# EmbodiedVision/diffsdfsim

Measured on AMD Instinct MI355X. Metric: sim steps/sec (fwd+bwd), 1024 batched 3D scenes x 8 SDF bodies, higher is better.
Workload: dtype f64

## Files before the change

diffsdfsim_amd/csrc/launchers.h:

```cpp
#pragma once
#include "dss_device.h"

#include "../../include/diffsdfsim_hip.h"

namespace dss {
int launch_find_contacts(const DssWorld &W, int *nc_out, int *body_out, int *face_out, double *abc_out,
                         double *geom_out, hipStream_t stream);
int launch_find_contacts_all(const DssWorld &W, int *nc_out, int *body_out, int *face_out, double *abc_out,
                             double *geom_out, hipStream_t stream);
int launch_find_contacts_box(const DssWorld &W, int *nc_out, int *body_out, int *face_out, double *abc_out,
                             double *geom_out, hipStream_t stream);
int launch_igr_rounds(const DssWorld &W, hipStream_t stream);
int launch_igr_list(const DssIgrNet &N, const double *pts, const int *lat_idx, const double *latents, int lat_stride,
                    const int *n_dev, int n_cap, int mode, double *sdf, double *grad, hipStream_t stream, int est);
int launch_igr_pair(const DssIgrNet &N, const double *pts_v, const int *lat_v, const int *n_v, double *sdf_v, const double *pts_g,
                    const int *lat_g, const int *n_g, double *sdf_g, double *grad_g, const double *latents, int lat_stride, int n_cap,
                    hipStream_t stream, int est_v, int est_g);
void launch_bwd_pre_all(const DssWorld &W, const DssAdjoint &A, hipStream_t stream);
int lcp_contact_backward_rows(const double *Mblk, const double *A, const double *cop, const int *cbody, const int *nc,
                              const int *active, int B, int nb, int neq, int maxc, int fric_dirs, const double *x,
                              const double *lam, const double *slack, const double *nu, const double *dl_dx, double *dMblk,
                              double *dpvec, double *dcop, double *dA, double *db, int rows, const int *slot, void *stream);
bool lcp_dense_group_fits(int nz, int nineq, int neq);
int launch_lcp_dense_group_forward(const double *Q, const double *p, const double *G, const double *h, const double *A, const double *b,
                                   const double *F, int B, int nz, int nineq, int neq, double eps, int not_improved_lim, int max_iter,
                                   int check_spd, double *zhat, double *lam, double *slack, double *nu, int *iters, int *status,
                                   hipStream_t stream);
int launch_lcp_dense_group_backward(const double *Q, const double *G, const double *A, const double *F, int B, int nz, int nineq, int neq,
                                    const double *zhat, const double *lam, const double *slack, const double *nu, const double *dl_dz,
                                    double *dQ, double *dp, double *dG, double *dh, double *dA, double *db, double *dF, hipStream_t stream);
}
```

diffsdfsim_amd/csrc/narrowphase.hip:

```cpp
#ifndef DSS_ALL_SHAPES
#define DSS_ALL_SHAPES 0
#endif
#ifndef DSS_BOX_ONLY
#define DSS_BOX_ONLY 0
#endif
#if !DSS_ALL_SHAPES && !DSS_BOX_ONLY
#define DSS_STAMPS np
#endif

#include "launchers.h"
#include "np_common.h"

namespace {
constexpr int NP_WAVES = 3;
constexpr int OV_RUN = 256;
constexpr int OV_NT = 256;
__global__ void __launch_bounds__(OV_NT) overlap_kernel(DssWorld W)
{
    __shared__ unsigned char s_ok[64 * 63 / 2];
    __shared__ unsigned char s_big[64];
    const int nb = W.nb, nup = nb * (nb - 1) / 2, np = npairs_of(nb);
    const int sc = blockIdx.x, tid = threadIdx.x, lane = tid & 63, wv = tid >> 6;
    if (!W.active[sc]) return;
    const bool few = (long)W.B * np <= 256L * NP_WAVES;
    if (tid < nb) {
        const int nf = W.mesh_nf[W.mesh_id[(size_t)sc * nb + tid]];
        s_big[tid] = nf > WAVE_ITEM_MAX_FACES || (few && nf > 2048);
    }
#if DSS_ALL_SHAPES
    __shared__ unsigned char s_igr[64];
    if (tid < nb) s_igr[tid] = W.shape_type[(size_t)sc * nb + tid] == DSS_SHAPE_IGR;
#endif
    for (int up = wv; up < nup; up += OV_NT / 64) {
        int i, j;
        upair_of(up, nb, i, j);
        int ok = !W.no_contact[i * nb + j];
        if (ok) {
            BodyD A, Bd;
            load_body(W, sc, i, A);
            load_body(W, sc, j, Bd);
            for (int dir = 0; dir < 2 && ok; ++dir) {
                const BodyD &src = dir ? Bd : A, &dst = dir ? A : Bd;
                const double s = dst.g.shape.scale;
                Region reg;
                region_of(src.g, dst.g, 1e-9, reg);
                const double *vbox = W.vch_box + (size_t)W.mesh_vch_off[src.mesh] * 6;
                const int nch = (src.nv + OV_RUN - 1) / OV_RUN;
                int found = 0;
                for (int cb0 = 0; cb0 < nch && !found; cb0 += 64) {
                    const int ch = cb0 + lane;
                    unsigned long long m = __ballot(ch < nch && box_hits(reg, vbox + (size_t)ch * 6));
                    while (m && !found) {
                        const int b = __ffsll((long long)m) - 1;
                        m &= m - 1;
                        int hit = 0;
#pragma unroll
                        for (int sub = 0; sub < OV_RUN / 64; ++sub) {
                            const int v = (cb0 + b) * OV_RUN + sub * 64 + lane;
                            if (v < src.nv) {
                                double p[3];
                                to_frame(src.g, dst.g, W.verts + (size_t)(src.voff + v) * 3, p);
                                hit |= (-s <= p[0] && p[0] <= s && -s <= p[1] && p[1] <= s && -s <= p[2] && p[2] <= s);
                            }
                        }
                        found = __ballot(hit) != 0ull;
                    }
                }
                ok = found;
            }
        }
        if (lane == 0) {
            s_ok[up] = (unsigned char)ok;
            W.ovl[((size_t)sc * nb + i) * nb + j] = ok;
            if (!ok) {
                W.pc_count[(size_t)sc * np + i * (nb - 1) + (j - 1)] = 0;
                W.pc_count[(size_t)sc * np + j * (nb - 1) + i] = 0;
            }
        }
    }
    __syncthreads();
    if (tid == 0) {
        int cnt[2] = {0, 0};
#if DSS_ALL_SHAPES
        int nig = 0;
        for (int up = 0, i = 0, j = 1; up < nup; ++up, upair_next(nb, i, j)) {
            if (s_ok[up] && (s_igr[i] || s_igr[j])) nig += 2;
        }
        if (nig) {
            int at = atomicAdd(W.n_pairs + 6, nig);
            for (int up = 0, i = 0, j = 1; up < nup; ++up, upair_next(nb, i, j)) {
                if (s_ok[up] && (s_igr[i] || s_igr[j])) {
                    s_ok[up] = 0;
                    if (W.igr_list && at + 2 <= W.igr_items_cap) {
                        W.igr_list[at++] = sc * np + i * (nb - 1) + (j - 1);
                        W.igr_list[at++] = sc * np + j * (nb - 1) + i;
                    } else atomicOr(W.overflow + sc, 32);
                }
            }
        }
#endif
        for (int up = 0, i = 0, j = 1; up < nup; ++up, upair_next(nb, i, j)) {
            if (s_ok[up]) { ++cnt[s_big[i] ? 0 : 1]; ++cnt[s_big[j] ? 0 : 1]; }
        }
        const int cap = W.B * np;
        const unsigned long long old = atomicAdd(reinterpret_cast<unsigned long long *>(W.n_pairs),
                                                 (unsigned long long)(unsigned)cnt[0] | ((unsigned long long)(unsigned)cnt[1] << 32));
        int at[2] = {(int)(old & 0xffffffffull), (int)(old >> 32)};
        for (int up = 0, i = 0, j = 1; up < nup; ++up, upair_next(nb, i, j)) {
            if (s_ok[up]) {
                const int li = s_big[i] ? 0 : 1, lj = s_big[j] ? 0 : 1;
                W.pair_list[(size_t)li * cap + at[li]++] = sc * np + i * (nb - 1) + (j - 1);
                W.pair_list[(size_t)lj * cap + at[lj]++] = sc * np + j * (nb - 1) + i;
            }
        }
    }
}

template <class G> __device__ int narrow_pair(const DssWorld &W, ScratchT<G> &S, int item, int slot_id)
{
    STAMP(0);
    item = dss_uniform(item); slot_id = dss_uniform(slot_id);
    const int np = npairs_of(W.nb);
    const int sc = item / np, dp = item % np, tid = G::tid();
    int a, b;
    pair_of(dp, W.nb, a, b);
    int *pc_count = W.pc_count + (size_t)sc * np + dp;
    BodyD A, Bd;
    load_body(W, sc, a, A);
    load_body(W, sc, b, Bd);
    const int MC = W.max_cand;
    int *__restrict__ cface = W.cand_face + (size_t)slot_id * 2 * MC, *__restrict__ kface = cface + MC;
    int *__restrict__ cstate = W.cand_state + (size_t)slot_id * MC;
    double *__restrict__ cb = W.cand_buf + (size_t)slot_id * DSS_CAND_FIELDS * MC;
    const double *__restrict__ m_verts = W.verts, *__restrict__ m_fcent = W.fcent;
    const int *__restrict__ m_faces = W.faces;
    const double sB = Bd.g.shape.scale;

    double R12[9], t12[3];
    pair_transform(A.g, Bd.g, R12, t12);

    int ncand = 0, over = 0;
    Region reg;
    region_of(A.g, Bd.g, 1e-9, reg);
    const double *fbox = W.fch_box + (size_t)W.mesh_fch_off[A.mesh] * 6;
    constexpr int RUN = 256;
    const int nch = (A.nf + RUN - 1) / RUN, lane = tid & 63, wv = tid >> 6;
    auto cull_face = [&](const double *c) -> int { return centroid_in_cube(R12, t12, c, sB); };
// ... 332 lines not shown
    DSS_KERNARG_REF(DssWorld, W, W_arg);
    __shared__ NpScratch S;
    __shared__ int s_item;
    const int cap = W.B * npairs_of(W.nb), seg = DEFERRED ? 2 : 0;
    {
        const int n = W.n_pairs[DEFERRED ? 4 : 0];
        const int *list = W.pair_list + (size_t)seg * cap;
        for (;;) {
            __syncthreads();
            if (threadIdx.x == 0) s_item = atomicAdd(W.n_pairs + (DEFERRED ? 5 : 2), 1);
            __syncthreads();
            const int it = s_item;
            if (it >= n) break;
            narrow_pair<BlockGroup>(W, S.blk, list[it], (int)blockIdx.x * BlockGroup::NW);
        }
    }
    if (DEFERRED) return;
    __syncthreads();
    const int n = W.n_pairs[1], lane = threadIdx.x & 63;
    const int *list = W.pair_list + cap;
    ScratchT<WaveGroup> &Sw = S.wav[threadIdx.x >> 6];
    for (;;) {
        int it = 0;
        if (lane == 0) it = atomicAdd(W.n_pairs + 3, 1);
        it = __shfl(it, 0);
        if (it >= n) break;
        const int item = list[it];
        if (narrow_pair<WaveGroup>(W, Sw, item, (int)(blockIdx.x * BlockGroup::NW + (threadIdx.x >> 6))) && lane == 0)
            W.pair_list[(size_t)2 * cap + atomicAdd(W.n_pairs + 4, 1)] = item;
        dss_wave_sync();
    }
}

__global__ void __launch_bounds__(64) compact_contacts_kernel(DssWorld W, int *nc_out, int *body_out, int *face_out,
                                                               double *abc_out, double *geom_out)
{
    constexpr int MAXSLOT = 64 * 63;
    __shared__ int s_off[MAXSLOT + 1];
    __shared__ short s_a[MAXSLOT], s_b[MAXSLOT];
    __shared__ unsigned char s_neg[MAXSLOT];
    const int sc = blockIdx.x, lane = threadIdx.x, nb = W.nb, np = npairs_of(nb), MP = W.max_pc, MX = W.maxc;
    if (!W.active[sc]) return;
    int run = 0;
    for (int base = 0; base < np; base += 64) {
        const int slot = base + lane;
        int cnt = 0, a = 0, b = 0;
        if (slot < np) {
            int i, j;
            upair_of(slot >> 1, nb, i, j);
            a = (slot & 1) ? j : i; b = (slot & 1) ? i : j;
            cnt = W.pc_count[(size_t)sc * np + a * (nb - 1) + (b < a ? b : b - 1)];
        }
        const int fwd = __shfl_up(cnt, 1, 64);
        if ((slot & 1) && fwd < 0) cnt = 0;
        if (slot < np) s_neg[slot] = cnt < 0;
        if (cnt < 0) cnt = -cnt;
        int incl = cnt;
        for (int d = 1; d < 64; d <<= 1) { const int o = __shfl_up(incl, d, 64); if (lane >= d) incl += o; }
        if (slot < np) { s_off[slot] = run + incl - cnt; s_a[slot] = (short)a; s_b[slot] = (short)b; }
        run += __shfl(incl, 63, 64);
    }
    if (lane == 0) s_off[np] = run;
    __syncthreads();
    const int total = run < MX ? run : MX;
    for (int o = lane; o < total; o += 64) {
        int lo = 0, hi = np;
        while (hi - lo > 1) { const int mid = (lo + hi) >> 1; if (s_off[mid] <= o) lo = mid; else hi = mid; }
        const int a = s_a[lo], b = s_b[lo], k = o - s_off[lo];
        const size_t dp = (size_t)sc * np + a * (nb - 1) + (b < a ? b : b - 1);
        const int *pf = W.pc_face + dp * MP;
        const double *pabc = W.pc_abc + dp * 3 * MP, *pg = W.pc_geom + dp * 10 * MP;
        const int face = s_neg[lo] ? -1 - pf[k] : pf[k];
        double abc[3], geo[10];
        for (int f = 0; f < 3; ++f) abc[f] = pabc[(size_t)f * MP + k];
        for (int f = 0; f < 10; ++f) geo[f] = pg[(size_t)f * MP + k];
        body_out[(size_t)sc * 2 * MX + o] = a;
        body_out[(size_t)sc * 2 * MX + MX + o] = b;
        face_out[(size_t)sc * MX + o] = face;
        for (int f = 0; f < 3; ++f) abc_out[((size_t)sc * 3 + f) * MX + o] = abc[f];
        for (int f = 0; f < 10; ++f) geom_out[((size_t)sc * 10 + f) * MX + o] = geo[f];
    }
    if (lane == 0) {
        if (run > MX) atomicOr(W.overflow + sc, 8);
        nc_out[sc] = total;
    }
}

}

namespace dss {
static inline int np_grid(int B, int nb)
{
    const long items = (long)B * nb * (nb - 1);
    return (int)(items < 256 * NP_WAVES ? items : 256 * NP_WAVES);
}
#if DSS_ALL_SHAPES
int launch_find_contacts_all(const DssWorld &W, int *nc_out, int *body_out, int *face_out, double *abc_out,
                             double *geom_out, hipStream_t stream)
{
#elif DSS_BOX_ONLY
int launch_find_contacts_box(const DssWorld &W, int *nc_out, int *body_out, int *face_out, double *abc_out,
                             double *geom_out, hipStream_t stream)
{
#else
int launch_find_contacts(const DssWorld &W, int *nc_out, int *body_out, int *face_out, double *abc_out,
                         double *geom_out, hipStream_t stream)
{
    if (W.shape_rare) return launch_find_contacts_all(W, nc_out, body_out, face_out, abc_out, geom_out, stream);
    if (W.shape_box) return launch_find_contacts_box(W, nc_out, body_out, face_out, abc_out, geom_out, stream);
#endif
    static_assert(BlockGroup::HCAP <= BlockGroup::BT * MAX_CPT && WaveGroup::HCAP <= WaveGroup::BT * MAX_CPT, "mover registers");
    if (W.max_cand < 1 || W.nb < 1) return DSS_E_UNSUPPORTED;
    if (W.nb < 2) {
        hipLaunchKernelGGL(compact_contacts_kernel, dim3(W.B), dim3(64), 0, stream, W, nc_out, body_out, face_out, abc_out, geom_out);
        return hipGetLastError() == hipSuccess ? DSS_OK : DSS_E_UNSUPPORTED;
    }
    const int nup = W.nb * (W.nb - 1) / 2, np = W.nb * (W.nb - 1);
    (void)hipMemsetAsync(W.n_pairs, 0, 8 * sizeof(int), stream);
    hipLaunchKernelGGL(overlap_kernel, dim3(W.B), dim3(OV_NT), 0, stream, W);
    const int grid = np_grid(W.B, W.nb);
    hipLaunchKernelGGL(narrowphase_kernel<false>, dim3(grid), dim3(NT), 0, stream, W);
    hipLaunchKernelGGL(narrowphase_kernel<true>, dim3(grid < 64 ? grid : 64), dim3(NT), 0, stream, W);
#if DSS_ALL_SHAPES
    if (W.igr_list) { const int rc = launch_igr_rounds(W, stream); if (rc) return rc; }
#endif
    hipLaunchKernelGGL(compact_contacts_kernel, dim3(W.B), dim3(64), 0, stream, W, nc_out, body_out, face_out, abc_out, geom_out);
    return hipGetLastError() == hipSuccess ? DSS_OK : DSS_E_UNSUPPORTED;
}
}

#if !DSS_ALL_SHAPES && !DSS_BOX_ONLY
extern "C" int dss_np_slots(int B, int nb) { return dss::np_grid(B, nb) * 4; }
#endif
```

diffsdfsim_amd/csrc/np_common.h:

```cpp
#pragma once
#include <math.h>
#include <stdlib.h>

#include "../../include/diffsdfsim_hip.h"
#include "contact_geom.h"
#include "diag_stamps.h"
#include "wave_utils.h"

namespace {
using namespace dss;

constexpr int NT = 256;
constexpr int MAX_CPT = 8;
constexpr int HULL3_MAX = 48;
constexpr int WAVE_ITEM_MAX_FACES = 1 << 30;
#define STAMP(i) DSS_STAMP(G::tid() == 0, (size_t)item * 8 + (i))

__device__ inline int npairs_of(int nb) { return nb * (nb - 1); }
__device__ inline void pair_of(int dp, int nb, int &a, int &b)
{
    a = dp / (nb - 1);
    const int r = dp % (nb - 1);
    b = r < a ? r : r + 1;
}
// ... 728 lines not shown
    return 0;
}
template <class G>
__device__ __noinline__ void emit_unfiltered(const DssWorld &W, int sc, int dp, int ncon, int over, const int *kface, const double *cb, int MC)
{
    const int np = npairs_of(W.nb), tid = G::tid(), MP = W.max_pc;
    int *pf = W.pc_face + ((size_t)sc * np + dp) * MP;
    double *pabc = W.pc_abc + ((size_t)sc * np + dp) * 3 * MP, *pg = W.pc_geom + ((size_t)sc * np + dp) * 10 * MP;
    int nout = ncon;
    if (nout > MP) { over |= 4; nout = MP; }
    for (int k = tid; k < nout; k += G::BT) {
        pf[k] = kface[k];
        for (int i = 0; i < 3; ++i) {
            pabc[(size_t)i * MP + k] = CB(F_CABC + i, k);
            pg[(size_t)i * MP + k] = CB(F_NORMAL + i, k);
            pg[(size_t)(3 + i) * MP + k] = CB(F_P1 + i, k);
            pg[(size_t)(6 + i) * MP + k] = CB(F_P2 + i, k);
        }
        pg[(size_t)9 * MP + k] = CB(F_PEN, k);
    }
    if (tid == 0) { W.pc_count[(size_t)sc * np + dp] = -nout; if (over) atomicOr(W.overflow + sc, over); }
}

template <class G>
__device__ __forceinline__ int filter_and_emit(const DssWorld &W, ScratchT<G> &S, int item, int sc, int dp, int ncon, int over,
                                               int *__restrict__ cface, int *__restrict__ kface, int *__restrict__ cstate,
                                               double *__restrict__ cb, int MC)
{
    const int np = npairs_of(W.nb), tid = G::tid();
    int *pc_count = W.pc_count + (size_t)sc * np + dp;
#include "np_filter_emit.inc"
}

}
```

diffsdfsim_amd/csrc/step.hip:

```cpp
#include <math.h>

#include "../../include/diffsdfsim_hip.h"
#include "contact_geom.h"
#include "launchers.h"
#include "wave_utils.h"

namespace {
using namespace dss;

__global__ void __launch_bounds__(64) begin_kernel(DssWorld W)
{
    const int sc = blockIdx.x * 64 + threadIdx.x;
    if (sc >= W.B) return;
    if (W.step_mask && !W.step_mask[sc]) { W.active[sc] = 0; return; }
    const double t = W.t[sc];
    W.t_end[sc] = t + W.dt;
    W.dt_try[sc] = (t + W.dt) - t;
    W.active[sc] = 1;
    if (W.had_contacts) W.had_contacts[sc] = 0;
    atomicAdd(W.n_active, 1);
}

__global__ void __launch_bounds__(64) assemble_kernel(DssWorld W)
{
    const int sc = blockIdx.x, lane = threadIdx.x, nb = W.nb, MX = W.maxc;
    if (!W.active[sc]) return;
    const int ND = W.fric_dirs / 2, NF = 3 * (1 + ND) + 8;
    double dt = W.dt_try[sc];
    if (W.toc_diff && W.toc[sc]) { const double l = W.last_dt[sc]; dt = -l + (l + dt); }
    if (lane == 0) { W.dt_use[sc] = dt; W.invalid[sc] = 0; }
    if (lane < nb) {
        const size_t bi = (size_t)sc * nb + lane;
        double ps[7], v[6];
        for (int i = 0; i < 7; ++i) { ps[i] = W.pose[bi * 7 + i]; W.pose0[bi * 7 + i] = ps[i]; }
        for (int i = 0; i < 6; ++i) { v[i] = W.vel[bi * 6 + i]; W.vel0[bi * 6 + i] = v[i]; }
        double Iw[9];
        world_inertia(ps, W.inertia + bi * 9, Iw);
// ... 19 lines not shown
        for (int i = 0; i < 3; ++i) { n[i] = g[(size_t)i * MX + c]; p1[i] = g[(size_t)(3 + i) * MX + c]; p2[i] = g[(size_t)(6 + i) * MX + c]; }
        friction_dirs(n, ND, D);
        for (int i = 0; i < 3; ++i) {
            cop[(size_t)i * MX + c] = n[i];
            for (int k = 0; k < ND; ++k) cop[(size_t)(3 * (k + 1) + i) * MX + c] = D[k][i];
        }
        const int o = 3 * (1 + ND);
        for (int i = 0; i < 3; ++i) { cop[(size_t)(o + i) * MX + c] = p1[i]; cop[(size_t)(o + 3 + i) * MX + c] = p2[i]; }
        const size_t i1 = (size_t)sc * nb + b1, i2 = (size_t)sc * nb + b2;
        cop[(size_t)(o + 6) * MX + c] = 0.5 * (W.fric[i1] + W.fric[i2]);
        const double *v1 = W.vel + i1 * 6, *v2 = W.vel + i2 * 6;
        double c1[3], c2[3], jv = 0.0;
        cross(p1, n, c1);
        cross(p2, n, c2);
        for (int i = 0; i < 3; ++i) jv += c1[i] * v1[i] + n[i] * v1[3 + i] - c2[i] * v2[i] - n[i] * v2[3 + i];
        cop[(size_t)(o + 7) * MX + c] = jv * (0.5 * (W.restitution[i1] + W.restitution[i2]));
    }
}

__global__ void __launch_bounds__(64) integrate_kernel(DssWorld W)
{
    const int sc = blockIdx.x, lane = threadIdx.x, nb = W.nb;
    if (!W.active[sc]) return;
    if (lane < nb) {
        const size_t bi = (size_t)sc * nb + lane;
        double v[6], out[7];
        for (int i = 0; i < 6; ++i) { v[i] = -W.x[(size_t)sc * 6 * nb + 6 * lane + i]; W.vel[bi * 6 + i] = v[i]; }
        const double dt = W.dt_use[sc];
        integrate_pose(W.pose0 + bi * 7, v, dt, out);
        for (int i = 0; i < 7; ++i) W.pose[bi * 7 + i] = out[i];
    }
}

struct NewContacts {
    int *nc, *body, *face;
    double *abc, *geom;
};

__global__ void __launch_bounds__(64) decide_kernel(DssWorld W, NewContacts N)
{
    const int sc = blockIdx.x, lane = threadIdx.x, nb = W.nb, MX = W.maxc;
    if (!W.active[sc]) return;
    if (lane == 0 && W.overflow[sc]) atomicOr(W.n_active, DSS_N_ACTIVE_OVERFLOW);
    const double dt_try = W.dt_try[sc];
    const bool tiny = !W.strict_no_pen && dt_try < W.dt / 1024.0;
    const bool accept = !W.invalid[sc] || tiny;
    if (accept) {
        const int nc_new = N.nc[sc], nc_old = W.nc[sc];
        __shared__ unsigned s_pairs[64 * 64 / 32];
        for (int w = lane; w < (nb * nb + 31) / 32; w += 64) s_pairs[w] = 0u;
        __syncthreads();
        for (int c = lane; c < nc_old; c += 64) {
            const int bit = W.c_body[(size_t)sc * 2 * MX + c] * nb + W.c_body[(size_t)sc * 2 * MX + MX + c];
            atomicOr(&s_pairs[bit >> 5], 1u << (bit & 31));
        }
        __syncthreads();
        int toc = 0;
        for (int c = lane; c < nc_new; c += 64) {
            const int a = N.body[(size_t)sc * 2 * MX + c], b = N.body[(size_t)sc * 2 * MX + MX + c];
            const int ab = a * nb + b, ba = b * nb + a;
            toc |= !(((s_pairs[ab >> 5] >> (ab & 31)) | (s_pairs[ba >> 5] >> (ba & 31))) & 1u);
        }
        toc = __ballot(toc) != 0ull;
        const bool escaped = W.invalid[sc] != 0;
        if (escaped) toc = W.toc[sc];
        const int slot = W.nsub[sc];
        if (W.tp_pose && slot >= W.max_sub && lane == 0) { atomicOr(W.overflow + sc, 16); atomicOr(W.n_active, DSS_N_ACTIVE_OVERFLOW); }
        if (W.tp_pose && slot < W.max_sub) {
            const size_t rec = (size_t)slot * W.B + sc;
            if (lane < nb) {
                for (int i = 0; i < 7; ++i) W.tp_pose[(rec * nb + lane) * 7 + i] = W.pose0[((size_t)sc * nb + lane) * 7 + i];
                for (int i = 0; i < 6; ++i) {
                    W.tp_vel[(rec * nb + lane) * 6 + i] = W.vel0[((size_t)sc * nb + lane) * 6 + i];
                    W.tp_x[rec * 6 * nb + 6 * lane + i] = W.x[(size_t)sc * 6 * nb + 6 * lane + i];
                }
            }
            if (lane < W.neq) W.tp_nu[rec * W.neq + lane] = W.nu[(size_t)sc * W.neq + lane];
            const int NR = W.fric_dirs + 2;
            for (int c = lane; c < nc_old; c += 64) {
                const int b1 = W.c_body[(size_t)sc * 2 * MX + c], b2 = W.c_body[(size_t)sc * 2 * MX + MX + c];
                const int face = W.c_face[(size_t)sc * MX + c];
                double abc[3], geo[10], lm[10], sl[10];
                for (int f = 0; f < 3; ++f) abc[f] = W.c_abc[((size_t)sc * 3 + f) * MX + c];
                for (int f = 0; f < 10; ++f) geo[f] = W.c_geom[((size_t)sc * 10 + f) * MX + c];
#pragma unroll
                for (int q = 0; q < 10; ++q)
                    if (q < NR) { lm[q] = W.lam[((size_t)sc * NR + q) * MX + c]; sl[q] = W.slack[((size_t)sc * NR + q) * MX + c]; }
                W.tp_body[rec * 2 * MX + c] = b1;
                W.tp_body[rec * 2 * MX + MX + c] = b2;
                W.tp_face[rec * MX + c] = face;
                for (int f = 0; f < 3; ++f) W.tp_abc[(rec * 3 + f) * MX + c] = abc[f];
                for (int f = 0; f < 10; ++f) W.tp_geom[(rec * 10 + f) * MX + c] = geo[f];
#pragma unroll
                for (int q = 0; q < 10; ++q)
                    if (q < NR) { W.tp_lam[(rec * NR + q) * MX + c] = lm[q]; W.tp_slack[(rec * NR + q) * MX + c] = sl[q]; }
            }
            if (lane == 0) {
                W.tp_dt[rec] = W.dt_use[sc]; W.tp_nc[rec] = nc_old;
                if (W.tp_t) W.tp_t[rec] = W.t[sc];
                W.tp_flags[rec] = ((W.toc_diff && toc && !escaped) ? 1 : 0) | ((W.toc_diff && W.toc[sc]) ? 2 : 0);
            }
        }
        __syncthreads();
        for (int c = lane; c < nc_new; c += 64) {
            const int b1 = N.body[(size_t)sc * 2 * MX + c], b2 = N.body[(size_t)sc * 2 * MX + MX + c], face = N.face[(size_t)sc * MX + c];
            double abc[3], geo[10];
            for (int f = 0; f < 3; ++f) abc[f] = N.abc[((size_t)sc * 3 + f) * MX + c];
            for (int f = 0; f < 10; ++f) geo[f] = N.geom[((size_t)sc * 10 + f) * MX + c];
            W.c_body[(size_t)sc * 2 * MX + c] = b1;
            W.c_body[(size_t)sc * 2 * MX + MX + c] = b2;
            W.c_face[(size_t)sc * MX + c] = face;
            for (int f = 0; f < 3; ++f) W.c_abc[((size_t)sc * 3 + f) * MX + c] = abc[f];
            for (int f = 0; f < 10; ++f) W.c_geom[((size_t)sc * 10 + f) * MX + c] = geo[f];
        }
        if (lane == 0) {
            W.nc[sc] = nc_new;
            if (W.had_contacts && nc_new > 0) W.had_contacts[sc] = 1;
            W.toc[sc] = toc;
            if (W.toc_diff && toc && !escaped) W.last_dt[sc] = W.dt_use[sc];
            W.nsub[sc] = slot + 1;
            const double t = W.t[sc] + dt_try;
            W.t[sc] = t;
            if (t < W.t_end[sc]) W.dt_try[sc] = W.t_end[sc] - t;
            else if (W.steps_left && W.steps_left[sc] > 1) {
                W.steps_left[sc] -= 1;
                W.t_end[sc] = t + W.dt;
                W.dt_try[sc] = (t + W.dt) - t;
                if (W.had_contacts) W.had_contacts[sc] = 0;
            }
            else { W.active[sc] = 0; atomicAdd(W.n_active, -1); }
        }
    } else {
        if (lane < nb) {
            const size_t bi = (size_t)sc * nb + lane;
            for (int i = 0; i < 7; ++i) W.pose[bi * 7 + i] = W.pose0[bi * 7 + i];
            for (int i = 0; i < 6; ++i) W.vel[bi * 6 + i] = W.vel0[bi * 6 + i];
        }
        if (lane == 0) W.dt_try[sc] = dt_try / 2.0;
    }
}

inline int check_world(const DssWorld *W)
{
    if (!W) return DSS_E_BADARG;
    if (W->B <= 0 || W->nb <= 0 || W->nb > 64 || W->maxc <= 0) return DSS_E_BADARG;
    if (W->fric_dirs != 4 && W->fric_dirs != 8) return DSS_E_BADARG;
    if (6 * W->nb + W->neq > 64) return DSS_E_UNSUPPORTED;
// ... 17 lines not shown
}

int dss_find_contacts(const DssWorld *W, void *stream)
{
    int rc = check_world(W);
    if (rc) return rc;
    return dss::launch_find_contacts(*W, W->nc, W->c_body, W->c_face, W->c_abc, W->c_geom, (hipStream_t)stream);
}

int dss_solve_dynamics(const DssWorld *W, void *lcp_workspace, size_t lcp_workspace_bytes, void *stream_)
{
    int rc = check_world(W);
    if (rc) return rc;
    hipLaunchKernelGGL(assemble_kernel, dim3(W->B), dim3(64), 0, (hipStream_t)stream_, *W);
    return dss_lcp_contact_forward(W->Mblk, W->pvec, W->Je, W->b_eq, W->cop, W->cop_body, W->nc, W->active, W->B, W->nb,
                                   W->neq, W->maxc, W->fric_dirs, 1e-12, 3, W->lcp_max_iter, W->x, W->lam, W->slack, W->nu,
                                   W->lcp_iters, W->lcp_status, lcp_workspace, lcp_workspace_bytes, stream_);
}

int dss_step_attempt(const DssWorld *W, void *lcp_workspace, size_t lcp_workspace_bytes, void *stream_)
{
    int rc = check_world(W);
    if (rc) return rc;
    hipStream_t stream = (hipStream_t)stream_;
    hipLaunchKernelGGL(assemble_kernel, dim3(W->B), dim3(64), 0, stream, *W);
    if (W->ev_lcp_start) (void)hipEventRecord((hipEvent_t)W->ev_lcp_start, stream);
    rc = dss_lcp_contact_forward(W->Mblk, W->pvec, W->Je, W->b_eq, W->cop, W->cop_body, W->nc,
                                 W->active, W->B, W->nb, W->neq, W->maxc, W->fric_dirs, 1e-12, 3, W->lcp_max_iter,
                                 W->x, W->lam, W->slack, W->nu, W->lcp_iters, W->lcp_status, lcp_workspace,
                                 lcp_workspace_bytes, stream_);
    if (W->ev_lcp_stop) (void)hipEventRecord((hipEvent_t)W->ev_lcp_stop, stream);
    if (rc) return rc;
    hipLaunchKernelGGL(integrate_kernel, dim3(W->B), dim3(64), 0, stream, *W);
    NewContacts N;
    N.nc = W->n_nc; N.body = W->n_body; N.face = W->n_face; N.abc = W->n_abc; N.geom = W->n_geom;
    if (W->ev_np_start) (void)hipEventRecord((hipEvent_t)W->ev_np_start, stream);
    rc = dss::launch_find_contacts(*W, N.nc, N.body, N.face, N.abc, N.geom, stream);
    if (W->ev_np_stop) (void)hipEventRecord((hipEvent_t)W->ev_np_stop, stream);
    if (rc) return rc;
    hipLaunchKernelGGL(decide_kernel, dim3(W->B), dim3(64), 0, stream, *W, N);
    return hipGetLastError() == hipSuccess ? DSS_OK : DSS_E_UNSUPPORTED;
}

}
```

diffsdfsim_amd/engine.py:

```python
import ctypes

import numpy as np

from . import world_abi as abi


class TorchBackend:

    def __init__(self, device="cuda"):
        import torch
        from . import _lib
        self.torch = torch
        self.device = torch.device(device)
        if self.device.type != "cuda" or not torch.cuda.is_available():
            raise _lib.HipLibraryError("BatchEngine needs a HIP device (got %s); there is no CPU fallback" % device)
        self.lib = _lib.lib()
        self._lib = _lib

    def zeros(self, shape, dtype):
        t = {np.float64: self.torch.float64, np.int32: self.torch.int32, np.uint8: self.torch.uint8}[dtype]
        return self.torch.zeros(shape, dtype=t, device=self.device)

    def from_numpy(self, a):
        return self.torch.as_tensor(np.ascontiguousarray(a)).to(self.device)
# ... 17 lines not shown
def default_vgrad(shape_type, prm, verts):
    verts = np.asarray(verts, np.float64)
    if shape_type in (abi.SHAPE_BOX_ROUNDED, abi.SHAPE_BRICK, abi.SHAPE_BOWL, abi.SHAPE_IGR, abi.SHAPE_GRID):
        return np.zeros_like(verts)
    if shape_type == abi.SHAPE_BOX:
        hd = np.asarray(prm, np.float64)[:3] / 2
        return np.where(np.abs(verts) == hd[None, :], 0.5 * np.sign(verts), 0.0)
    if shape_type == abi.SHAPE_CYLINDER:
        rho = np.maximum(np.hypot(verts[:, 0], verts[:, 1]), 1e-300)
        hh = float(prm[1]) / 2
        side = rho > 0.5 * float(prm[0])
        return np.stack([np.where(side, verts[:, 0] / rho, 0.0), np.where(side, verts[:, 1] / rho, 0.0),
                         np.where(verts[:, 2] == hh, 0.5, np.where(verts[:, 2] == -hh, -0.5, 0.0))], axis=1)
    return verts / float(prm[0])


def mesh_table(meshes, vgrads=None):
    voff, nv, foff, nf, V, F, C, R = [], [], [], [], [], [], [], []
    fch, vch, fch_off, vch_off = [], [], [], []
    nfc = nvc = 0
    vo = fo = 0
    for verts, faces in meshes:
        verts = np.asarray(verts, np.float64); faces = np.asarray(faces, np.int64)
        voff.append(vo); nv.append(len(verts)); foff.append(fo); nf.append(len(faces))
        tri = verts[faces]
        cen = tri.mean(axis=1)
        rad = np.linalg.norm(cen[:, None, :] - tri, axis=2).max(axis=1)
        V.append(verts); F.append(faces.astype(np.int32)); C.append(cen); R.append(rad)
        vo += len(verts); fo += len(faces)
        fch_off.append(nfc); vch_off.append(nvc)
        for k in range(0, len(faces), CHUNK):
            c, r = cen[k:k + CHUNK], rad[k:k + CHUNK, None]
            fch.append(np.concatenate([(c - r).min(0), (c + r).max(0)]))
        for k in range(0, len(verts), CHUNK):
            fv = verts[k:k + CHUNK]
            vch.append(np.concatenate([fv.min(0), fv.max(0)]))
        nfc, nvc = len(fch), len(vch)
    i32 = lambda x: np.asarray(x, np.int32)
    out = dict(mesh_voff=i32(voff), mesh_nv=i32(nv), mesh_foff=i32(foff), mesh_nf=i32(nf),
               fch_box=np.stack(fch), vch_box=np.stack(vch), mesh_fch_off=i32(fch_off), mesh_vch_off=i32(vch_off),
               verts=np.concatenate(V), faces=np.concatenate(F), fcent=np.concatenate(C), frad=np.concatenate(R))
    out["vgrad"] = np.concatenate([np.asarray(g, np.float64) for g in vgrads]) if vgrads is not None else np.zeros_like(out["verts"])
    return out


def check_igr_spec(spec):
    from . import igr
    B, nb = np.asarray(spec["pose"]).shape[:2]
    if spec.get("igr_net") is None:
        raise ValueError("a body of shape_type SHAPE_IGR needs spec['igr_net'] (diffsdfsim_amd.igr.pack_weights)")
    shape = igr.packed_shape(spec["igr_net"])
    if shape not in igr.SHAPES:
        raise NotImplementedError("no kernels are built for a network of width %d and latent size %d" % tuple(shape))
    lat = spec.get("igr_latent")
    if shape == igr.SHAPES[0]:
        if lat is not None:
            raise ValueError("spec['igr_latent'] goes with the 7 -> 8 x 256 -> 1 network; the 5 -> 8 x 128 -> 1 network's "
                             "2-number latent code is shape_prm[..., :2]")
        return None
    if lat is None:
        raise ValueError("the 7 -> 8 x 256 -> 1 network's 4-number latent code does not fit the 3 shape parameters per body: "
                         "give spec['igr_latent'] [B, nb, %d]" % abi.IGR_LATENT_MAX)
    lat = np.asarray(lat, np.float64)
    if lat.shape != (B, nb, abi.IGR_LATENT_MAX):
        raise ValueError("spec['igr_latent'] has shape %s, expected %s" % (lat.shape, (B, nb, abi.IGR_LATENT_MAX)))
    return lat


class BatchEngine:
# ... 229 lines not shown
```

diffsdfsim_amd/world_abi.py:

```python
import ctypes

import numpy as np

ABI_VERSION = 4
CAND_FIELDS = 28
CSCR_ROWS = 56
N_ACTIVE_OVERFLOW = 1 << 30
SHAPE_BOX, SHAPE_SPHERE, SHAPE_CYLINDER, SHAPE_BOX_ROUNDED, SHAPE_BRICK, SHAPE_BOWL, SHAPE_IGR, SHAPE_GRID = 0, 1, 2, 3, 4, 5, 6, 7
IGR_HDR, IGR_ROUNDS = 16, 42
IGR_LATENT_MAX = 4

_I, _D, _P = ctypes.c_int, ctypes.c_double, ctypes.c_void_p

PROTOTYPES = {
    "dss_abi_version": ("i", ""),
    "dss_lcp_dense_workspace_bytes": ("z", "iiii"), "dss_lcp_dense_forward": ("i", "pppppppiiiidiiipppppppzp"),
    "dss_lcp_dense_backward": ("i", "ppppiiiipppppppppppppzp"),
    "dss_lcp_contact_workspace_bytes": ("z", "iiiii"), "dss_lcp_contact_forward": ("i", "ppppppppiiiiidiipppppppzp"),
    "dss_lcp_contact_backward": ("i", "ppppppiiiiippppppppppp"),
    "dss_world_sizeof": ("z", ""), "dss_np_slots": ("i", "ii"), "dss_step_begin": ("i", "pp"), "dss_step_attempt": ("i", "ppzp"),
    "dss_solve_dynamics": ("i", "ppzp"), "dss_find_contacts": ("i", "pp"),
    "dss_adjoint_sizeof": ("z", ""), "dss_step_backward": ("i", "ppp"),
    "dss_igr_packed_doubles": ("z", ""), "dss_igr_query_list": ("i", "ppppipiippp"), "dss_igr_query": ("i", "ppppppppippp"),
    "dss_igr_query_latent_grad": ("i", "ppppppppippp"),
# ... 75 lines not shown
NP_DTYPE = {"pd": np.float64, "pi": np.int32, "pb": np.uint8}


def igr_shapes(items_cap, qcap, max_cand, B=None, nb=None, maxc=None):
    extra = {}
    if B is not None:
        cap = B * 2 * maxc
        extra = {"igr_latent": (B, nb, IGR_LATENT_MAX), "g_latent": (B, nb, IGR_LATENT_MAX), "igr_bw_n": (1,), "igr_bw_idx": (B, 2, maxc),
                 "igr_bw_pts": (cap, 3), "igr_bw_lat": (cap,), "igr_bw_sdf": (2, cap), "igr_bw_grad": (cap * (3 + IGR_LATENT_MAX),)}
    return {
        **extra,
        "igr_list": (items_cap,), "igr_hdr": (items_cap, IGR_HDR), "igr_cface": (items_cap, 3, max_cand),
        "igr_cstate": (items_cap, max_cand), "igr_cbuf": (items_cap, CAND_FIELDS, max_cand),
        "igr_qpts": (4, qcap, 3), "igr_qlat": (4, qcap), "igr_qtag": (4, qcap), "igr_qsdf": (4, qcap), "igr_qgrad": (2, qcap, 3),
        "igr_qn": (2 * (IGR_ROUNDS + 2),),
    }


def array_shapes(B, nb, neq, maxc, fd, max_cand, max_pc, max_sub, nmesh, NV, NF, np_slots, NFC=1, NVC=1):
    npair = nb * (nb - 1)
    NR = fd + 2
    NFc = 3 * (1 + fd // 2) + 8
    nz = 6 * nb
    s = {
        "pose": (B, nb, 7), "vel": (B, nb, 6), "mass": (B, nb), "inertia": (B, nb, 9), "restitution": (B, nb),
        "fric": (B, nb), "fext": (B, nb, 6), "shape_type": (B, nb), "shape_prm": (B, nb, 3), "shape_aux": (B, nb), "mesh_id": (B, nb),
        "no_contact": (nb, nb), "mesh_voff": (nmesh,), "mesh_nv": (nmesh,), "mesh_foff": (nmesh,), "mesh_nf": (nmesh,),
        "verts": (NV, 3), "faces": (NF, 3), "fcent": (NF, 3), "frad": (NF,), "vgrad": (NV, 3),
        "fch_box": (NFC, 6), "vch_box": (NVC, 6), "mesh_fch_off": (nmesh,), "mesh_vch_off": (nmesh,),
        "Je": (B, max(neq, 1), nz), "b_eq": (B, max(neq, 1)),
        "t": (B,), "t_end": (B,), "dt_try": (B,), "last_dt": (B,), "dt_use": (B,),
        "active": (B,), "had_contacts": (B,), "toc": (B,), "nsub": (B,), "n_active": (1,),
        "nc": (B,), "c_body": (B, 2, maxc), "c_face": (B, maxc), "c_abc": (B, 3, maxc), "c_geom": (B, 10, maxc),
        "n_nc": (B,), "n_body": (B, 2, maxc), "n_face": (B, maxc), "n_abc": (B, 3, maxc), "n_geom": (B, 10, maxc),
        "pose0": (B, nb, 7), "vel0": (B, nb, 6),
        "Mblk": (B, nb, 6, 6), "pvec": (B, nz), "cop": (B, NFc, maxc), "x": (B, nz), "lam": (B, NR, maxc),
        "slack": (B, NR, maxc), "nu": (B, max(neq, 1)), "cop_body": (B, 2, maxc), "lcp_iters": (B,), "lcp_status": (B,),
        "ovl": (B, nb, nb), "pair_list": (3 * B * npair,), "n_pairs": (8,), "invalid": (B,), "overflow": (B,),
        "pc_count": (B, npair), "pc_stats": (B, npair, 2), "pc_face": (B, npair, max_pc), "pc_abc": (B, npair, 3, max_pc),
        "pc_geom": (B, npair, 10, max_pc),
        "cand_face": (np_slots, 2, max_cand), "cand_state": (np_slots, max_cand), "cand_buf": (np_slots, CAND_FIELDS, max_cand),
    }
    if max_sub > 0:
        s.update({
            "tp_pose": (max_sub, B, nb, 7), "tp_vel": (max_sub, B, nb, 6), "tp_dt": (max_sub, B), "tp_x": (max_sub, B, nz),
            "tp_lam": (max_sub, B, NR, maxc), "tp_slack": (max_sub, B, NR, maxc), "tp_nu": (max_sub, B, max(neq, 1)),
            "tp_abc": (max_sub, B, 3, maxc), "tp_geom": (max_sub, B, 10, maxc),
            "tp_nc": (max_sub, B), "tp_body": (max_sub, B, 2, maxc), "tp_face": (max_sub, B, maxc), "tp_flags": (max_sub, B), "tp_t": (max_sub, B),
        })
    return s


ADJ_FIELDS = [
    ("a_pose", "pd"), ("a_vel", "pd"), ("a_geom", "pd"), ("a_last_dt", "pd"), ("a_dt", "pd"),
    ("g_mass", "pd"), ("g_inertia", "pd"), ("g_rest", "pd"), ("g_fric", "pd"), ("g_fext", "pd"), ("g_prm", "pd"), ("g_verts", "pd"),
    ("cur_slot", "pi"), ("lo_slot", "pi"), ("bw_active", "pi"),
    ("a_x", "pd"), ("dMblk", "pd"), ("dpvec", "pd"), ("dcop", "pd"), ("cscr", "pd"), ("bw_nc", "pi"),
    ("igr_bw_n", "pi"), ("igr_bw_idx", "pi"), ("igr_bw_pts", "pd"), ("igr_bw_lat", "pi"), ("igr_bw_sdf", "pd"), ("igr_bw_grad", "pd"),
    ("g_latent", "pd"),
]


class DssAdjoint(ctypes.Structure):
    _fields_ = [(n, _P) for n, k in ADJ_FIELDS]


def adjoint_shapes(B, nb, maxc, fd, NV=1, igr=False, latent_table=False):
# ... 13 lines not shown
```

Before: 528.2.

## Fuse contact compaction into decide kernel and parallelize overlap pair emission

The step path no longer runs a separate compaction kernel into temporary n_* buffers. The decide kernel now gathers per-pair contact counts and copies contacts directly into the committed contact arrays, which removes one launch and a full round trip through scratch memory. The overlap kernel's serial single-thread pair-list emission is replaced with a wave-wide packed-count reduction and prefix scan. Vertex chunk boxes also gain a whole-mesh bounding box that is tested first, so disjoint pairs skip the chunk loop. In exchange, decide_kernel carries a large shared scratch block, which may lower occupancy, and the packed 12-bit counters assume per-scene counts stay below 4096.

```diff
diff --git a/diffsdfsim_amd/csrc/launchers.h b/diffsdfsim_amd/csrc/launchers.h
--- a/diffsdfsim_amd/csrc/launchers.h
+++ b/diffsdfsim_amd/csrc/launchers.h
@@ -4,12 +4,11 @@
 #include "../../include/diffsdfsim_hip.h"
 
 namespace dss {
+int launch_detect(const DssWorld &W, hipStream_t stream);
+int launch_detect_all(const DssWorld &W, hipStream_t stream);
+int launch_detect_box(const DssWorld &W, hipStream_t stream);
 int launch_find_contacts(const DssWorld &W, int *nc_out, int *body_out, int *face_out, double *abc_out,
                          double *geom_out, hipStream_t stream);
-int launch_find_contacts_all(const DssWorld &W, int *nc_out, int *body_out, int *face_out, double *abc_out,
-                             double *geom_out, hipStream_t stream);
-int launch_find_contacts_box(const DssWorld &W, int *nc_out, int *body_out, int *face_out, double *abc_out,
-                             double *geom_out, hipStream_t stream);
 int launch_igr_rounds(const DssWorld &W, hipStream_t stream);
 int launch_igr_list(const DssIgrNet &N, const double *pts, const int *lat_idx, const double *latents, int lat_stride,
                     const int *n_dev, int n_cap, int mode, double *sdf, double *grad, hipStream_t stream, int est);
diff --git a/diffsdfsim_amd/csrc/narrowphase.hip b/diffsdfsim_amd/csrc/narrowphase.hip
--- a/diffsdfsim_amd/csrc/narrowphase.hip
+++ b/diffsdfsim_amd/csrc/narrowphase.hip
@@ -44,8 +44,8 @@
                 const double s = dst.g.shape.scale;
                 Region reg;
                 region_of(src.g, dst.g, 1e-9, reg);
-                const double *vbox = W.vch_box + (size_t)W.mesh_vch_off[src.mesh] * 6;
-                const int nch = (src.nv + OV_RUN - 1) / OV_RUN;
+                const double *mbox = W.vch_box + (size_t)W.mesh_vch_off[src.mesh] * 6, *vbox = mbox + 6;
+                const int nch = box_hits(reg, mbox) ? (src.nv + OV_RUN - 1) / OV_RUN : 0;
                 int found = 0;
                 for (int cb0 = 0; cb0 < nch && !found; cb0 += 64) {
                     const int ch = cb0 + lane;
@@ -79,40 +79,57 @@
         }
     }
     __syncthreads();
-    if (tid == 0) {
-        int cnt[2] = {0, 0};
+    if (wv != 0) return;
+    const int cap = W.B * np;
+    auto entries = [&](int up, int &i, int &j) -> unsigned {
+        if (up >= nup || !s_ok[up]) return 0u;
+        upair_of(up, nb, i, j);
 #if DSS_ALL_SHAPES
-        int nig = 0;
-        for (int up = 0, i = 0, j = 1; up < nup; ++up, upair_next(nb, i, j)) {
-            if (s_ok[up] && (s_igr[i] || s_igr[j])) nig += 2;
-        }
-        if (nig) {
-            int at = atomicAdd(W.n_pairs + 6, nig);
-            for (int up = 0, i = 0, j = 1; up < nup; ++up, upair_next(nb, i, j)) {
-                if (s_ok[up] && (s_igr[i] || s_igr[j])) {
-                    s_ok[up] = 0;
-                    if (W.igr_list && at + 2 <= W.igr_items_cap) {
-                        W.igr_list[at++] = sc * np + i * (nb - 1) + (j - 1);
-                        W.igr_list[at++] = sc * np + j * (nb - 1) + i;
-                    } else atomicOr(W.overflow + sc, 32);
-                }
-            }
-        }
-#endif
-        for (int up = 0, i = 0, j = 1; up < nup; ++up, upair_next(nb, i, j)) {
-            if (s_ok[up]) { ++cnt[s_big[i] ? 0 : 1]; ++cnt[s_big[j] ? 0 : 1]; }
-        }
-        const int cap = W.B * np;
+        if (s_igr[i] || s_igr[j]) return 2u << 24;
+#endif
+        return (1u << (s_big[i] ? 0 : 12)) + (1u << (s_big[j] ? 0 : 12));
+    };
+    unsigned tot = 0u;
+    for (int base = 0; base < nup; base += 64) { int i, j; tot += entries(base + lane, i, j); }
+    int cnt[3];
+    for (int l = 0; l < 3; ++l) {
+        int c = (int)((tot >> (12 * l)) & 0xfffu);
+        for (int o = 32; o > 0; o >>= 1) c += __shfl_xor(c, o, 64);
+        cnt[l] = c;
+    }
+    int at[3] = {0, 0, 0};
+    if (lane == 0) {
+#if DSS_ALL_SHAPES
+        if (cnt[2]) at[2] = atomicAdd(W.n_pairs + 6, cnt[2]);
+#endif
         const unsigned long long old = atomicAdd(reinterpret_cast<unsigned long long *>(W.n_pairs),
                                                  (unsigned long long)(unsigned)cnt[0] | ((unsigned long long)(unsigned)cnt[1] << 32));
-        int at[2] = {(int)(old & 0xffffffffull), (int)(old >> 32)};
-        for (int up = 0, i = 0, j = 1; up < nup; ++up, upair_next(nb, i, j)) {
-            if (s_ok[up]) {
+        at[0] = (int)(old & 0xffffffffull); at[1] = (int)(old >> 32);
+    }
+    for (int l = 0; l < 3; ++l) at[l] = __shfl(at[l], 0, 64);
+    for (int base = 0; base < nup; base += 64) {
+        int i = 0, j = 0;
+        const unsigned mine = entries(base + lane, i, j);
+        unsigned incl = mine;
+        for (int d = 1; d < 64; d <<= 1) { const unsigned o = __shfl_up(incl, d, 64); if (lane >= d) incl += o; }
+        const unsigned excl = incl - mine, all = __shfl(incl, 63, 64);
+        if (mine) {
+            const int item_ij = sc * np + i * (nb - 1) + (j - 1), item_ji = sc * np + j * (nb - 1) + i;
+#if DSS_ALL_SHAPES
+            if (mine >> 24) {
+                const int o = at[2] + (int)(excl >> 24);
+                if (W.igr_list && o + 2 <= W.igr_items_cap) { W.igr_list[o] = item_ij; W.igr_list[o + 1] = item_ji; }
+                else atomicOr(W.overflow + sc, 32);
+            } else
+#endif
+            {
                 const int li = s_big[i] ? 0 : 1, lj = s_big[j] ? 0 : 1;
-                W.pair_list[(size_t)li * cap + at[li]++] = sc * np + i * (nb - 1) + (j - 1);
-                W.pair_list[(size_t)lj * cap + at[lj]++] = sc * np + j * (nb - 1) + i;
-            }
-        }
+                int o[2] = {at[0] + (int)(excl & 0xfffu), at[1] + (int)((excl >> 12) & 0xfffu)};
+                W.pair_list[(size_t)li * cap + o[li]++] = item_ij;
+                W.pair_list[(size_t)lj * cap + o[lj]] = item_ji;
+            }
+        }
+        at[0] += (int)(all & 0xfffu); at[1] += (int)((all >> 12) & 0xfffu); at[2] += (int)(all >> 24);
     }
 }
 
@@ -511,59 +528,21 @@
     }
 }
 
+#if !DSS_ALL_SHAPES && !DSS_BOX_ONLY
 __global__ void __launch_bounds__(64) compact_contacts_kernel(DssWorld W, int *nc_out, int *body_out, int *face_out,
                                                                double *abc_out, double *geom_out)
 {
-    constexpr int MAXSLOT = 64 * 63;
-    __shared__ int s_off[MAXSLOT + 1];
-    __shared__ short s_a[MAXSLOT], s_b[MAXSLOT];
-    __shared__ unsigned char s_neg[MAXSLOT];
-    const int sc = blockIdx.x, lane = threadIdx.x, nb = W.nb, np = npairs_of(nb), MP = W.max_pc, MX = W.maxc;
+    __shared__ GatherScratch S;
+    const int sc = blockIdx.x;
     if (!W.active[sc]) return;
-    int run = 0;
-    for (int base = 0; base < np; base += 64) {
-        const int slot = base + lane;
-        int cnt = 0, a = 0, b = 0;
-        if (slot < np) {
-            int i, j;
-            upair_of(slot >> 1, nb, i, j);
-            a = (slot & 1) ? j : i; b = (slot & 1) ? i : j;
-            cnt = W.pc_count[(size_t)sc * np + a * (nb - 1) + (b < a ? b : b - 1)];
-        }
-        const int fwd = __shfl_up(cnt, 1, 64);
-        if ((slot & 1) && fwd < 0) cnt = 0;
-        if (slot < np) s_neg[slot] = cnt < 0;
-        if (cnt < 0) cnt = -cnt;
-        int incl = cnt;
-        for (int d = 1; d < 64; d <<= 1) { const int o = __shfl_up(incl, d, 64); if (lane >= d) incl += o; }
-        if (slot < np) { s_off[slot] = run + incl - cnt; s_a[slot] = (short)a; s_b[slot] = (short)b; }
-        run += __shfl(incl, 63, 64);
-    }
-    if (lane == 0) s_off[np] = run;
-    __syncthreads();
-    const int total = run < MX ? run : MX;
-    for (int o = lane; o < total; o += 64) {
-        int lo = 0, hi = np;
-        while (hi - lo > 1) { const int mid = (lo + hi) >> 1; if (s_off[mid] <= o) lo = mid; else hi = mid; }
-        const int a = s_a[lo], b = s_b[lo], k = o - s_off[lo];
-        const size_t dp = (size_t)sc * np + a * (nb - 1) + (b < a ? b : b - 1);
-        const int *pf = W.pc_face + dp * MP;
-        const double *pabc = W.pc_abc + dp * 3 * MP, *pg = W.pc_geom + dp * 10 * MP;
-        const int face = s_neg[lo] ? -1 - pf[k] : pf[k];
-        double abc[3], geo[10];
-        for (int f = 0; f < 3; ++f) abc[f] = pabc[(size_t)f * MP + k];
-        for (int f = 0; f < 10; ++f) geo[f] = pg[(size_t)f * MP + k];
-        body_out[(size_t)sc * 2 * MX + o] = a;
-        body_out[(size_t)sc * 2 * MX + MX + o] = b;
-        face_out[(size_t)sc * MX + o] = face;
-        for (int f = 0; f < 3; ++f) abc_out[((size_t)sc * 3 + f) * MX + o] = abc[f];
-        for (int f = 0; f < 10; ++f) geom_out[((size_t)sc * 10 + f) * MX + o] = geo[f];
-    }
-    if (lane == 0) {
-        if (run > MX) atomicOr(W.overflow + sc, 8);
+    const int run = gather_slots(W, sc, S), total = run < W.maxc ? run : W.maxc;
+    gather_contacts(W, sc, S, total, body_out, face_out, abc_out, geom_out);
+    if (threadIdx.x == 0) {
+        if (run > W.maxc) atomicOr(W.overflow + sc, 8);
         nc_out[sc] = total;
     }
 }
+#endif
 
 }
 
@@ -574,27 +553,20 @@
     return (int)(items < 256 * NP_WAVES ? items : 256 * NP_WAVES);
 }
 #if DSS_ALL_SHAPES
-int launch_find_contacts_all(const DssWorld &W, int *nc_out, int *body_out, int *face_out, double *abc_out,
-                             double *geom_out, hipStream_t stream)
+int launch_detect_all(const DssWorld &W, hipStream_t stream)
 {
 #elif DSS_BOX_ONLY
-int launch_find_contacts_box(const DssWorld &W, int *nc_out, int *body_out, int *face_out, double *abc_out,
-                             double *geom_out, hipStream_t stream)
+int launch_detect_box(const DssWorld &W, hipStream_t stream)
 {
 #else
-int launch_find_contacts(const DssWorld &W, int *nc_out, int *body_out, int *face_out, double *abc_out,
-                         double *geom_out, hipStream_t stream)
-{
-    if (W.shape_rare) return launch_find_contacts_all(W, nc_out, body_out, face_out, abc_out, geom_out, stream);
-    if (W.shape_box) return launch_find_contacts_box(W, nc_out, body_out, face_out, abc_out, geom_out, stream);
+int launch_detect(const DssWorld &W, hipStream_t stream)
+{
+    if (W.shape_rare) return launch_detect_all(W, stream);
+    if (W.shape_box) return launch_detect_box(W, stream);
 #endif
     static_assert(BlockGroup::HCAP <= BlockGroup::BT * MAX_CPT && WaveGroup::HCAP <= WaveGroup::BT * MAX_CPT, "mover registers");
     if (W.max_cand < 1 || W.nb < 1) return DSS_E_UNSUPPORTED;
-    if (W.nb < 2) {
-        hipLaunchKernelGGL(compact_contacts_kernel, dim3(W.B), dim3(64), 0, stream, W, nc_out, body_out, face_out, abc_out, geom_out);
-        return hipGetLastError() == hipSuccess ? DSS_OK : DSS_E_UNSUPPORTED;
-    }
-    const int nup = W.nb * (W.nb - 1) / 2, np = W.nb * (W.nb - 1);
+    if (W.nb < 2) return DSS_OK;
     (void)hipMemsetAsync(W.n_pairs, 0, 8 * sizeof(int), stream);
     hipLaunchKernelGGL(overlap_kernel, dim3(W.B), dim3(OV_NT), 0, stream, W);
     const int grid = np_grid(W.B, W.nb);
@@ -603,9 +575,18 @@
 #if DSS_ALL_SHAPES
     if (W.igr_list) { const int rc = launch_igr_rounds(W, stream); if (rc) return rc; }
 #endif
+    return hipGetLastError() == hipSuccess ? DSS_OK : DSS_E_UNSUPPORTED;
+}
+#if !DSS_ALL_SHAPES && !DSS_BOX_ONLY
+int launch_find_contacts(const DssWorld &W, int *nc_out, int *body_out, int *face_out, double *abc_out,
+                         double *geom_out, hipStream_t stream)
+{
+    const int rc = launch_detect(W, stream);
+    if (rc) return rc;
     hipLaunchKernelGGL(compact_contacts_kernel, dim3(W.B), dim3(64), 0, stream, W, nc_out, body_out, face_out, abc_out, geom_out);
     return hipGetLastError() == hipSuccess ? DSS_OK : DSS_E_UNSUPPORTED;
 }
+#endif
 }
 
 #if !DSS_ALL_SHAPES && !DSS_BOX_ONLY
diff --git a/diffsdfsim_amd/csrc/np_common.h b/diffsdfsim_amd/csrc/np_common.h
--- a/diffsdfsim_amd/csrc/np_common.h
+++ b/diffsdfsim_amd/csrc/np_common.h
@@ -784,4 +784,59 @@
 #include "np_filter_emit.inc"
 }
 
-}
+constexpr int GATHER_MAXSLOT = 64 * 63;
+struct GatherScratch {
+    int off[GATHER_MAXSLOT + 1];
+    short a[GATHER_MAXSLOT], b[GATHER_MAXSLOT];
+    unsigned char neg[GATHER_MAXSLOT];
+};
+__device__ inline int gather_slots(const DssWorld &W, int sc, GatherScratch &S)
+{
+    const int lane = threadIdx.x, nb = W.nb, np = npairs_of(nb);
+    int run = 0;
+    for (int base = 0; base < np; base += 64) {
+        const int slot = base + lane;
+        int cnt = 0, a = 0, b = 0;
+        if (slot < np) {
+            int i, j;
+            upair_of(slot >> 1, nb, i, j);
+            a = (slot & 1) ? j : i; b = (slot & 1) ? i : j;
+            cnt = W.pc_count[(size_t)sc * np + a * (nb - 1) + (b < a ? b : b - 1)];
+        }
+        const int fwd = __shfl_up(cnt, 1, 64);
+        if ((slot & 1) && fwd < 0) cnt = 0;
+        if (slot < np) S.neg[slot] = cnt < 0;
+        if (cnt < 0) cnt = -cnt;
+        int incl = cnt;
+        for (int d = 1; d < 64; d <<= 1) { const int o = __shfl_up(incl, d, 64); if (lane >= d) incl += o; }
+        if (slot < np) { S.off[slot] = run + incl - cnt; S.a[slot] = (short)a; S.b[slot] = (short)b; }
+        run += __shfl(incl, 63, 64);
+    }
+    if (lane == 0) S.off[np] = run;
+    __syncthreads();
+    return run;
+}
+__device__ inline void gather_contacts(const DssWorld &W, int sc, const GatherScratch &S, int total, int *body_out, int *face_out,
+                                       double *abc_out, double *geom_out)
+{
+    const int lane = threadIdx.x, nb = W.nb, np = npairs_of(nb), MP = W.max_pc, MX = W.maxc;
+    for (int o = lane; o < total; o += 64) {
+        int lo = 0, hi = np;
+        while (hi - lo > 1) { const int mid = (lo + hi) >> 1; if (S.off[mid] <= o) lo = mid; else hi = mid; }
+        const int a = S.a[lo], b = S.b[lo], k = o - S.off[lo];
+        const size_t dp = (size_t)sc * np + a * (nb - 1) + (b < a ? b : b - 1);
+        const int *pf = W.pc_face + dp * MP;
+        const double *pabc = W.pc_abc + dp * 3 * MP, *pg = W.pc_geom + dp * 10 * MP;
+        const int face = S.neg[lo] ? -1 - pf[k] : pf[k];
+        double abc[3], geo[10];
+        for (int f = 0; f < 3; ++f) abc[f] = pabc[(size_t)f * MP + k];
+        for (int f = 0; f < 10; ++f) geo[f] = pg[(size_t)f * MP + k];
+        body_out[(size_t)sc * 2 * MX + o] = a;
+        body_out[(size_t)sc * 2 * MX + MX + o] = b;
+        face_out[(size_t)sc * MX + o] = face;
+        for (int f = 0; f < 3; ++f) abc_out[((size_t)sc * 3 + f) * MX + o] = abc[f];
+        for (int f = 0; f < 10; ++f) geom_out[((size_t)sc * 10 + f) * MX + o] = geo[f];
+    }
+}
+
+}
diff --git a/diffsdfsim_amd/csrc/step.hip b/diffsdfsim_amd/csrc/step.hip
--- a/diffsdfsim_amd/csrc/step.hip
+++ b/diffsdfsim_amd/csrc/step.hip
@@ -3,6 +3,7 @@
 #include "../../include/diffsdfsim_hip.h"
 #include "contact_geom.h"
 #include "launchers.h"
+#include "np_common.h"
 #include "wave_utils.h"
 
 namespace {
@@ -88,21 +89,22 @@
     }
 }
 
-struct NewContacts {
-    int *nc, *body, *face;
-    double *abc, *geom;
-};
-
-__global__ void __launch_bounds__(64) decide_kernel(DssWorld W, NewContacts N)
-{
+__global__ void __launch_bounds__(64) decide_kernel(DssWorld W)
+{
+    __shared__ GatherScratch S;
     const int sc = blockIdx.x, lane = threadIdx.x, nb = W.nb, MX = W.maxc;
     if (!W.active[sc]) return;
-    if (lane == 0 && W.overflow[sc]) atomicOr(W.n_active, DSS_N_ACTIVE_OVERFLOW);
+    const int nc_run = gather_slots(W, sc, S), nc_new = nc_run < MX ? nc_run : MX;
+    if (lane == 0) {
+        int over = W.overflow[sc];
+        if (nc_run > MX) { atomicOr(W.overflow + sc, 8); over |= 8; }
+        if (over) atomicOr(W.n_active, DSS_N_ACTIVE_OVERFLOW);
+    }
     const double dt_try = W.dt_try[sc];
     const bool tiny = !W.strict_no_pen && dt_try < W.dt / 1024.0;
     const bool accept = !W.invalid[sc] || tiny;
     if (accept) {
-        const int nc_new = N.nc[sc], nc_old = W.nc[sc];
+        const int nc_old = W.nc[sc];
         __shared__ unsigned s_pairs[64 * 64 / 32];
         for (int w = lane; w < (nb * nb + 31) / 32; w += 64) s_pairs[w] = 0u;
         __syncthreads();
@@ -112,8 +114,9 @@
         }
         __syncthreads();
         int toc = 0;
-        for (int c = lane; c < nc_new; c += 64) {
-            const int a = N.body[(size_t)sc * 2 * MX + c], b = N.body[(size_t)sc * 2 * MX + MX + c];
+        for (int slot = lane; slot < npairs_of(nb); slot += 64) {
+            if (!(S.off[slot] < nc_new && S.off[slot + 1] > S.off[slot])) continue;
+            const int a = S.a[slot], b = S.b[slot];
             const int ab = a * nb + b, ba = b * nb + a;
             toc |= !(((s_pairs[ab >> 5] >> (ab & 31)) | (s_pairs[ba >> 5] >> (ba & 31))) & 1u);
         }
@@ -158,17 +161,7 @@
             }
         }
         __syncthreads();
-        for (int c = lane; c < nc_new; c += 64) {
-            const int b1 = N.body[(size_t)sc * 2 * MX + c], b2 = N.body[(size_t)sc * 2 * MX + MX + c], face = N.face[(size_t)sc * MX + c];
-            double abc[3], geo[10];
-            for (int f = 0; f < 3; ++f) abc[f] = N.abc[((size_t)sc * 3 + f) * MX + c];
-            for (int f = 0; f < 10; ++f) geo[f] = N.geom[((size_t)sc * 10 + f) * MX + c];
-            W.c_body[(size_t)sc * 2 * MX + c] = b1;
-            W.c_body[(size_t)sc * 2 * MX + MX + c] = b2;
-            W.c_face[(size_t)sc * MX + c] = face;
-            for (int f = 0; f < 3; ++f) W.c_abc[((size_t)sc * 3 + f) * MX + c] = abc[f];
-            for (int f = 0; f < 10; ++f) W.c_geom[((size_t)sc * 10 + f) * MX + c] = geo[f];
-        }
+        gather_contacts(W, sc, S, nc_new, W.c_body, W.c_face, W.c_abc, W.c_geom);
         if (lane == 0) {
             W.nc[sc] = nc_new;
             if (W.had_contacts && nc_new > 0) W.had_contacts[sc] = 1;
@@ -252,13 +245,11 @@
     if (W->ev_lcp_stop) (void)hipEventRecord((hipEvent_t)W->ev_lcp_stop, stream);
     if (rc) return rc;
     hipLaunchKernelGGL(integrate_kernel, dim3(W->B), dim3(64), 0, stream, *W);
-    NewContacts N;
-    N.nc = W->n_nc; N.body = W->n_body; N.face = W->n_face; N.abc = W->n_abc; N.geom = W->n_geom;
     if (W->ev_np_start) (void)hipEventRecord((hipEvent_t)W->ev_np_start, stream);
-    rc = dss::launch_find_contacts(*W, N.nc, N.body, N.face, N.abc, N.geom, stream);
+    rc = dss::launch_detect(*W, stream);
     if (W->ev_np_stop) (void)hipEventRecord((hipEvent_t)W->ev_np_stop, stream);
     if (rc) return rc;
-    hipLaunchKernelGGL(decide_kernel, dim3(W->B), dim3(64), 0, stream, *W, N);
+    hipLaunchKernelGGL(decide_kernel, dim3(W->B), dim3(64), 0, stream, *W);
     return hipGetLastError() == hipSuccess ? DSS_OK : DSS_E_UNSUPPORTED;
 }
 
diff --git a/diffsdfsim_amd/engine.py b/diffsdfsim_amd/engine.py
--- a/diffsdfsim_amd/engine.py
+++ b/diffsdfsim_amd/engine.py
@@ -73,9 +73,11 @@
         for k in range(0, len(faces), CHUNK):
             c, r = cen[k:k + CHUNK], rad[k:k + CHUNK, None]
             fch.append(np.concatenate([(c - r).min(0), (c + r).max(0)]))
-        for k in range(0, len(verts), CHUNK):
-            fv = verts[k:k + CHUNK]
-            vch.append(np.concatenate([fv.min(0), fv.max(0)]))
+        runs = [verts[k:k + CHUNK] for k in range(0, len(verts), CHUNK)]
+        boxes = [np.concatenate([fv.min(0), fv.max(0)]) for fv in runs]
+        lo = np.min([b[:3] for b in boxes], axis=0) if boxes else np.full(3, np.inf)
+        hi = np.max([b[3:] for b in boxes], axis=0) if boxes else np.full(3, -np.inf)
+        vch += [np.concatenate([lo, hi])] + boxes
         nfc, nvc = len(fch), len(vch)
     i32 = lambda x: np.asarray(x, np.int32)
     out = dict(mesh_voff=i32(voff), mesh_nv=i32(nv), mesh_foff=i32(foff), mesh_nf=i32(nf),
diff --git a/diffsdfsim_amd/world_abi.py b/diffsdfsim_amd/world_abi.py
--- a/diffsdfsim_amd/world_abi.py
+++ b/diffsdfsim_amd/world_abi.py
@@ -131,7 +131,6 @@
         "t": (B,), "t_end": (B,), "dt_try": (B,), "last_dt": (B,), "dt_use": (B,),
         "active": (B,), "had_contacts": (B,), "toc": (B,), "nsub": (B,), "n_active": (1,),
         "nc": (B,), "c_body": (B, 2, maxc), "c_face": (B, maxc), "c_abc": (B, 3, maxc), "c_geom": (B, 10, maxc),
-        "n_nc": (B,), "n_body": (B, 2, maxc), "n_face": (B, maxc), "n_abc": (B, 3, maxc), "n_geom": (B, 10, maxc),
         "pose0": (B, nb, 7), "vel0": (B, nb, 6),
         "Mblk": (B, nb, 6, 6), "pvec": (B, nz), "cop": (B, NFc, maxc), "x": (B, nz), "lam": (B, NR, maxc),
         "slack": (B, NR, maxc), "nu": (B, max(neq, 1)), "cop_body": (B, 2, maxc), "lcp_iters": (B,), "lcp_status": (B,),
```

Measured after the change: 528.9 (median of 2 runs). Within noise of the previous version (+0.1%).
